# swishersnaaake/sexy-raytracer

Measured on AMD Instinct MI355X. Metric: Msamples/s (WxHxspp/s), 720p masterchief @5k spp, higher is better.
Workload: dtype f32; 1 GPU; masterchief_720p_5000spp; scene=masterchief, width=1280, height=720, spp=5000, max_bounce=4, seed=1, spp_chunks=625, tree=reference, traversal=faithful (bvh.h order), parallelism=tiles8x8 interleaved over 1 rank(s), 1 gather (none)

## Files before the change

sexy-raytracer_amd/csrc/srt_wavefront.hip:

```cpp
#include "srt_path.h"
#include "srt_launch.h"
#include "srt_wf_links.h"
#include "srt_wf_rings.h"

#define WF_BLOCK 1024
#define WF_SET_OF(mask) std::integral_constant<uint32_t, (mask)>()
#define WF_CTX_BYTES 128
#define WF_CTL_LIVE 28
#define WF_CTL_ABORT 29
#define WF_CTL_WORDS 64
#define WF_PEND_MISS 0
#define WF_PEND_TERMINAL 2

namespace {
enum { W_NODE = 0, W_PRIM = 1, W_SWAP = 2, W_SERVE = 3 };

__device__ __forceinline__ void bufStore4(Rsrc r, int off, float4 v) {
  u32x4 u;
  u.x = __float_as_uint(v.x); u.y = __float_as_uint(v.y); u.z = __float_as_uint(v.z); u.w = __float_as_uint(v.w);
  __builtin_amdgcn_raw_buffer_store_b128(u, r, off, 0, 0);
}
__device__ __forceinline__ void bufStore1(Rsrc r, int off, uint32_t v) { __builtin_amdgcn_raw_buffer_store_b32(v, r, off, 0, 0); }
typedef float f32x4 __attribute__((ext_vector_type(4)));
typedef __attribute__((address_space(3))) const f32x4 LdsVec4;
__device__ __forceinline__ uint32_t bufLoad1(Rsrc r, int off) { return __builtin_amdgcn_raw_buffer_load_b32(r, off, 0, 0); }
}

#define WF_PROF_KINDS 12
template <bool SINGLE, bool PROFILE, bool HYBRID, bool COUNT, bool MOMENTS = false>
__global__ __launch_bounds__(WF_BLOCK, 4) void srt_render_wf_kernel(const RenderArgs a) {
  static_assert(!(MOMENTS && (COUNT || PROFILE)), "the moments instances neither count nor profile");

  constexpr int32_t DONE = HYBRID ? -(1 << 29) : SRT_WF_DONE;
  constexpr int32_t DONE_PAIR = HYBRID ? (int32_t)0x80000000 : SRT_WF_DONE;
  typedef typename std::conditional<HYBRID, int32_t, uint16_t>::type PrimSlot;
  extern __shared__ int32_t lds[];
  const DevScene& sc = a.scene;
  char* const ldsTree = reinterpret_cast<char*>(lds);
  const int resident = HYBRID ? sc.wfResident : sc.numNodes;
  const int treeBytes = resident * 32;
  int32_t* const ctl = reinterpret_cast<int32_t*>(ldsTree + treeBytes);
  const int RCAP = a.wfRingCap, POOL = a.wfPoolSize;
  uint16_t* const ringSlots = reinterpret_cast<uint16_t*>(ctl + WF_CTL_WORDS);
  float* const hitT = reinterpret_cast<float*>(ringSlots + WF_RINGS * RCAP);
  PrimSlot* const hitPrim = reinterpret_cast<PrimSlot*>(hitT + POOL);
  const int lane = threadIdx.x & 63;
  const unsigned long long laneBelow = (1ull << lane) - 1ull;
  const uint64_t seedMixed = mix64(a.seed);
  const V3 background = ld3(a.background);
  const Rsrc rsNodes = makeRsrc(HYBRID ? sc.nodesWf : sc.nodes, sc.numNodes * 32);
  const Rsrc rsTris = makeRsrc(sc.triTest, HYBRID ? sc.numTris * 48 : 0);
  const Rsrc rsFast = makeRsrc(sc.triFast, HYBRID ? 0 : sc.numTris * 64);
  const Rsrc rsSpheres = makeRsrc(sc.spheres, sc.numSpheres * 48);
  const Rsrc rsTexels = makeRsrc(sc.texels, sc.texelBytes);
  const Rsrc rsClass = makeRsrc(sc.primClass, sc.numPrimClass);
  const Rsrc rsSecond = makeRsrc(sc.primSecond, HYBRID ? sc.numPrimClass * 4 : 0);
  const Rsrc rsPool = makeRsrc(a.wfPool + (size_t)blockIdx.x * POOL * WF_CTX_BYTES, POOL * WF_CTX_BYTES);
  const int hiLevels = a.maxBounce > 4 ? a.maxBounce - 4 : 0;
  const Rsrc rsAttHi = makeRsrc(a.wfAttHi + (size_t)blockIdx.x * 3 * hiLevels * POOL, 3 * hiLevels * POOL * 4);
  const bool singleRoot = SINGLE || sc.numWorld == 1;
  auto worldRef = [&](int k) {
    if (HYBRID) return sc.worldWf[k];
    return srtWfRootWord(sc.world[k]);
  };
  const SrtWfRingGeom ringGeom = {a.wfRingCap, a.wfRingShift, a.wfRingMul3};

  {
    float4* dst = reinterpret_cast<float4*>(ldsTree);
    for (int i = threadIdx.x; i < resident * 2; i += WF_BLOCK) {
      float4 v = bufLoad4(rsNodes, 16 * i);
      if (!HYBRID) {
        const int32_t thread = sc.nodeThread[i >> 1];
        v.w = __int_as_float((i & 1) ? srtWfMissWord(thread) : srtWfHitWord(__float_as_int(v.w), thread));
      }
      dst[i] = v;
    }
    for (int i = threadIdx.x; i < WF_CTL_WORDS; i += WF_BLOCK) ctl[i] = 0;
    for (int i = threadIdx.x; i < WF_RINGS * RCAP; i += WF_BLOCK) ringSlots[i] = 0;
    __syncthreads();
    for (int id = threadIdx.x; id < POOL; id += WF_BLOCK) ringSlots[WF_RING_NEWITEM * RCAP + id] = (uint16_t)(id + 1);
    if (threadIdx.x == 0) {
      ctl[WF_CTL_TAIL(WF_RING_NEWITEM)] = POOL;
      ctl[WF_CTL_LIVE] = POOL;
    }
    if (threadIdx.x < 16) ctl[threadIdx.x] = (int)(blockIdx.x % (unsigned)a.numQueues);
    __syncthreads();
  }
  int32_t* const waveQueue = ctl + (threadIdx.x >> 6);
  const int qHome = (int)(blockIdx.x % (unsigned)a.numQueues);
  const int unitItems = a.unitTiles * a.sppChunks * SRT_TILE_PIXELS;
  auto queueEnd = [&](int q) { return (q < a.numUnits ? (a.numUnits - q + a.numQueues - 1) / a.numQueues : 0) * unitItems; };

  auto raiseAbort = [&]() {
    if (__hip_atomic_exchange(&ctl[WF_CTL_ABORT], 1, __ATOMIC_RELAXED, WF_WG) == 0 && a.wfError) atomicAdd(a.wfError, 1);
  };
  auto enqueue = [&](auto set, int ring, int id) {
    if constexpr (HYBRID)
      srtWfEnqueueGeneric(ctl, ringSlots, ringGeom, lane, laneBelow, ring, id, raiseAbort);
    else
      srtWfEnqueue<decltype(set)::value>(ctl, ringSlots, ringGeom, lane, ring, id, raiseAbort);
  };

  int path = -1;
  int cur = DONE, hitRef = DONE, w = 0;
  int32_t link = DONE_PAIR;
  Ray ray;
  ray.o = ray.d = mk(0.0f, 0.0f, 0.0f);
  ray.time = 0.0f;
  float closest = SRT_INF, rayA = 0.0f, slabTol = SRT_INF;
  V3 rcpD = mk(0.0f, 0.0f, 0.0f), negOR = mk(0.0f, 0.0f, 0.0f);
  auto atNode = [&]() { return cur >= 0; };
  auto atPrim = [&]() { return (uint32_t)cur > (uint32_t)DONE; };
  unsigned long long cnt[8] = {0, 0, 0, 0, 0, 0, 0, 0};
  uint32_t walk0[4] = {0, 0, 0, 0};
  int aovPixel = -1;
  auto popNext = [&]() {
    int next;
    if (HYBRID) {
      const int follows = link & 3;
      next = link >> 2;
      if (follows == 1) next = cur - 2;
      if (follows == 2) next = (int)__builtin_amdgcn_raw_buffer_load_b32(rsSecond, (~cur) << 2, 0, 0);
      link &= ~3;
    } else {
      next = srtWfLeafHasSecond(cur) ? srtWfLeafRest(cur) : link;
    }
    if (!SINGLE && !singleRoot && next == DONE && ++w < sc.numWorld) {
      next = worldRef(w);
      link = DONE_PAIR;
    }
    cur = next;
  };
  auto startTraversal = [&]() {
    if constexpr (COUNT) {
      cnt[1]++;
      for (int k = 0; k < 4; ++k) walk0[k] = (uint32_t)cnt[2 + k];
    }
    rayA = lenSq(ray.d);
    const bool certified = (sc.fastDivScene != 0) & fastDivOperandOk(ray.o.x, ray.d.x) & fastDivOperandOk(ray.o.y, ray.d.y) &
                           fastDivOperandOk(ray.o.z, ray.d.z);
    rcpD = mk(refinedRcp(ray.d.x), refinedRcp(ray.d.y), refinedRcp(ray.d.z));
    slabSetup(ray.o, rcpD, certified, negOR, slabTol);
    closest = SRT_INF;
    hitRef = DONE;
    link = DONE_PAIR;
    w = 0;
    cur = worldRef(0);
  };
  auto cameraRayInto = [&](int at, uint32_t pxy, int s, float m1 = 0.0f, float m2 = 0.0f) {
    const int px = (int)(pxy & 0xffffu), py = (int)(pxy >> 16);
    Pcg rng;
    rng.key(seedMixed, (uint32_t)(py * a.imageWidth + px), (uint32_t)s);
    const float u = ((float)px + rng.uniform()) / (float)(a.imageWidth - 1);
    const float v = ((float)(a.imageHeight - py) + rng.uniform()) / (float)(a.imageHeight - 1);
    Ray r;
    const DevCamera cam = cameraFromKernarg();
    cameraRay(cam, u, v, rng, r);
    if constexpr (COUNT) cnt[0]++;
    bufStore4(rsPool, at, make_float4(r.o.x, r.o.y, r.o.z, r.time));
    bufStore4(rsPool, at + 16, make_float4(r.d.x, r.d.y, r.d.z, MOMENTS ? m1 : 0.0f));
    u32x4 Cn;
    Cn.x = (uint32_t)rng.state;
    Cn.y = (uint32_t)(rng.state >> 32);
    Cn.z = MOMENTS ? __float_as_uint(m2) : 0u;
    Cn.w = 0;
    __builtin_amdgcn_raw_buffer_store_b128(Cn, rsPool, at + 32, 0, 0);
  };

  int idleTrips = 0;
  uint32_t tick = 0;
  unsigned long long pCyc[WF_PROF_KINDS], pRuns[WF_PROF_KINDS], pLanes[WF_PROF_KINDS], pSched = 0;
  unsigned long long pSaw[8] = {0, 0, 0, 0, 0, 0, 0, 0};
  for (int k = 0; k < WF_PROF_KINDS; ++k) pCyc[k] = pRuns[k] = pLanes[k] = 0;
  const unsigned long long pStart = PROFILE ? clock64() : 0;
  unsigned long long pT = pStart;
  auto prof = [&](int kind, int lanes) {
    if (PROFILE) {
      const unsigned long long now = clock64();
      pCyc[kind] += now - pT;
      pRuns[kind]++;
      pLanes[kind] += lanes;
      pT = now;
    }
  };
  auto primStep = [&]() -> int {
    int nNodes;
      for (int round = 0; round < SRT_PRIM_ROUNDS; ++round) {
        if (round > 0 && __popcll(__ballot(atPrim())) < a.primAgainMin) break;
        if (PROFILE) {
          pRuns[1]++;
          pLanes[1] += __popcll(__ballot(atPrim()));
        }
        if (atPrim()) {
          const int ref = HYBRID ? cur : srtWfLeafFirst(cur);
          const int pr = ~ref;
          float t;
          bool ok;
          if (pr & 1) {
            if constexpr (COUNT) cnt[5]++;
            const int off = (pr >> 1) * 48;
            const float4 s0 = bufLoad4(rsSpheres, off), s1 = bufLoad4(rsSpheres, off + 16);
            V3 center = mk(s0.x, s0.y, s0.z);
            if (__float_as_int(s1.w) & (1 << 30)) {
              const float4 s2 = bufLoad4(rsSpheres, off + 32);
              center = center + ((ray.time - s2.x) / (s2.y - s2.x)) * (mk(s1.x, s1.y, s1.z) - center);
            }
            ok = sphereHitV(center, s0.w, ray, rayA, a.tMin, closest, t);
          } else {
            if constexpr (COUNT) cnt[4]++;
            if constexpr (HYBRID) {
              const int off = (pr >> 1) * 48;
              ok = triHitV<false>(bufLoad4(rsTris, off), bufLoad4(rsTris, off + 16), bufLoad4(rsTris, off + 32), ray, a.tMin, closest, t);
            } else {
              bool unsure;
              const int off = (pr >> 1) * 64;
              ok = srtTriHitCert(bufLoad4(rsFast, off), bufLoad4(rsFast, off + 16), bufLoad4(rsFast, off + 32), bufLoad4(rsFast, off + 48),
                                 triRay(ray), a.tMin, sc.triWMax, t, unsure);
              const unsigned long long mu = __ballot(unsure);
              if (PROFILE) {
                pRuns[11] += __popcll(mu);
                pCyc[11] += mu != 0 ? 1 : 0;
              }
              if (mu != 0) {
                if (unsure) {
                  const Rsrc rsExact = makeRsrc(sc.triTest, sc.numTris * 48);
                  const int at = (pr >> 1) * 48;
                  ok = triHitV<false>(bufLoad4(rsExact, at), bufLoad4(rsExact, at + 16), bufLoad4(rsExact, at + 32), ray, a.tMin, closest, t);
                }
              }
            }
          }
          if (ok) {
            closest = t;
            hitRef = ref;
          }
          popNext();
        }
      }
      nNodes = __popcll(__ballot(atNode()));
      if (PROFILE) {
        const unsigned long long now = clock64();
        pCyc[1] += now - pT;
        pT = now;
      }
      return nNodes;
  };
  auto nodeBurst = [&](int nNodes) -> int {
      const int keep = (nNodes * a.keepEighths) >> 3;
      int budget = a.nodeBurst, left;
      auto visit = [&](const float4 n0, const float4 n1) {
        bool undecided;
        bool hitBox = boxHitApprox<true>(n0, n1, rcpD, negOR, slabTol, a.tMin, closest, undecided);
        if (PROFILE) {
          const unsigned long long mu = __ballot(undecided);
          pLanes[8] += __popcll(mu);
          pLanes[7] += mu != 0 ? 1 : 0;
        }
        if (undecided) hitBox = boxHit(n0, n1, ray, a.tMin, closest);
        if constexpr (COUNT) {
          cnt[2]++;
          if (hitBox) cnt[3]++;
        }
        link = __float_as_int(n1.w);
        cur = hitBox ? __float_as_int(n0.w) : (HYBRID ? link >> 2 : link);
        if (!SINGLE && !singleRoot && cur == DONE && ++w < sc.numWorld) {
          cur = worldRef(w);
          link = DONE_PAIR;
        }
      };
      auto nodeVisit = [&](bool mine) {
        const bool here = HYBRID ? mine && (uint32_t)cur < (uint32_t)resident : cur >= 0;
        if (PROFILE) {
          pRuns[0]++;
          pLanes[0] += __popcll(__ballot(here));
        }
        if (here) {
          if constexpr (HYBRID) {
            const char* rec = ldsTree + (cur << 5);
            visit(*reinterpret_cast<const float4*>(rec), *reinterpret_cast<const float4*>(rec + 16));
          } else {
            const LdsVec4* rec = (const LdsVec4*)(uintptr_t)(uint32_t)cur;
            const f32x4 n0 = rec[0], n1 = rec[1];
            visit(make_float4(n0.x, n0.y, n0.z, n0.w), make_float4(n1.x, n1.y, n1.z, n1.w));
          }
        }
      };
      do {
        if (HYBRID) {
          const bool far = cur >= resident;
          float4 g0, g1;
          if (far) {
            g0 = bufLoad4(rsNodes, cur << 5);
            g1 = bufLoad4(rsNodes, (cur << 5) + 16);
          }
          if (a.wfFarRounds > 1) nodeVisit(!far);
          if (a.wfFarRounds > 2) nodeVisit(!far);
          if (a.wfFarRounds > 3) nodeVisit(!far);
          const bool near = !far && (uint32_t)cur < (uint32_t)resident;
          if (near) {
            const char* rec = ldsTree + (cur << 5);
            g0 = *reinterpret_cast<const float4*>(rec);
            g1 = *reinterpret_cast<const float4*>(rec + 16);
          }
          const unsigned long long f0 = PROFILE ? clock64() : 0;
          if (far || near) visit(g0, g1);
          if (PROFILE) {
            pRuns[10]++;
            pLanes[10] += __popcll(__ballot(far));
            pLanes[11] += __popcll(__ballot(near));
            pCyc[10] += clock64() - f0;
          }
        } else {
#pragma unroll
          for (int u = 0; u < SRT_NODE_UNROLL; ++u) nodeVisit(true);
        }
        budget -= HYBRID ? a.wfFarRounds : SRT_NODE_UNROLL;
        left = __popcll(__ballot(atNode()));
      } while (budget > 0 && left >= keep);
      if (PROFILE) {
        const unsigned long long now = clock64();
        pCyc[0] += now - pT;
        pT = now;
      }
      return left;
  };
  auto swapStep = [&]() {
      const bool fin = cur == DONE && path >= 0;
      const bool hit = fin && hitRef != DONE;
      const bool need = path < 0 || fin;
      const unsigned long long mNeed = __ballot(need);
      int id = -1;
      int cls = 0;
      if (hit) cls = (int)__builtin_amdgcn_raw_buffer_load_b8(rsClass, ~hitRef, 0, 0);
      const unsigned long long q0 = PROFILE ? clock64() : 0;
      if (mNeed != 0) {
        if constexpr (HYBRID)
          srtWfClaimGeneric(ctl, ringSlots, ringGeom, lane, laneBelow, WF_RING_READY, mNeed, __popcll(mNeed), 1, id, raiseAbort);
        else
          srtWfClaim(ctl, ringSlots, ringGeom, lane, WF_RING_READY, need, mNeed, __popcll(mNeed), 1, id, raiseAbort);
      }
      const unsigned long long q1 = PROFILE ? clock64() : 0;
      float4 A = make_float4(0.0f, 0.0f, 0.0f, 0.0f), B = A;
      if (id >= 0) {
        A = bufLoad4(rsPool, id << 7);
        B = bufLoad4(rsPool, (id << 7) + 16);
      }
      if (hit) {
        __hip_atomic_store(&hitT[path], closest, __ATOMIC_RELAXED, WF_WG);
        __hip_atomic_store(&hitPrim[path], (PrimSlot)hitRef, __ATOMIC_RELAXED, WF_WG);
      }
      asm volatile("" ::: "memory");
      enqueue(WF_SET_OF(WF_SET(WF_RING_RESTART) | WF_SET(WF_RING_HIT) | WF_SET(WF_RING_HIT + 1) | WF_SET(WF_RING_HIT + 2)),
              !fin ? -1 : (hit ? WF_RING_HIT + cls : WF_RING_RESTART), path);
      if constexpr (COUNT) {
        if (fin && aovPixel >= 0) {
          SrtAovRecord r;
          r.o[0] = ray.o.x; r.o[1] = ray.o.y; r.o[2] = ray.o.z;
          r.d[0] = ray.d.x; r.d[1] = ray.d.y; r.d[2] = ray.d.z;
          r.time = ray.time;
          r.valid = 1;
          r.prim = SRT_NO_HIT;
          r.t = 0.0f;
          if (hitRef != DONE) {
            const int pr = ~hitRef;
            r.prim = (pr & 1) ? sc.sphPrimId[pr >> 1] : sc.triPrimId[pr >> 1];
            r.t = closest;
          }
          r.nodeVisits = (int32_t)((uint32_t)cnt[2] - walk0[0]);
          r.boxPasses = (int32_t)((uint32_t)cnt[3] - walk0[1]);
          r.triTests = (int32_t)((uint32_t)cnt[4] - walk0[2]);
          r.sphereTests = (int32_t)((uint32_t)cnt[5] - walk0[3]);
          r.pad[0] = r.pad[1] = 0;
          a.aov[aovPixel] = r;
        }
      }
      if (fin) {
        path = -1;
        hitRef = DONE;
      }
      const unsigned long long q2 = PROFILE ? clock64() : 0;
      if (id >= 0) {
        ray.o = mk(A.x, A.y, A.z);
        ray.d = mk(B.x, B.y, B.z);
        ray.time = A.w;
        path = id;
        startTraversal();
        if constexpr (COUNT) {
          aovPixel = -1;
          if (a.aov) {
            const uint32_t cw = bufLoad1(rsPool, (id << 7) + 44);
            const u32x4 E = __builtin_amdgcn_raw_buffer_load_b128(rsPool, (id << 7) + 64, 0, 0);
            const int px = (int)(E.w & 0xffffu), py = (int)(E.w >> 16);
            if ((int)(cw & 0xffu) == a.aovDepth && (int)E.y == a.sampleFirst) aovPixel = py * a.imageWidth + px;
          }
        }
      }
      if (PROFILE) {
        const unsigned long long q3 = clock64();
        pSaw[5] += q1 - q0;
        pSaw[6] += q2 - q1;
        pSaw[7] += q3 - q2;
      }
      prof(2, __popcll(__ballot(fin)) + __popcll(__ballot(id >= 0)));
  };
  auto serveStep = [&](int bestRing, int serveAtLeast) -> int {
      int id;
      const unsigned long long h0 = PROFILE ? clock64() : 0;
      int k;
      if constexpr (HYBRID)
        k = srtWfClaimGeneric(ctl, ringSlots, ringGeom, lane, laneBelow, bestRing, ~0ull, 64, serveAtLeast, id, raiseAbort);
      else
        k = srtWfClaimAll(ctl, ringSlots, ringGeom, lane, bestRing, 64, serveAtLeast, id, raiseAbort);
      if (k == 0) {
        prof(8, 0);
        return 0;
      }
      const int at = id << 7;
      if (bestRing >= WF_RING_HIT && bestRing < WF_RING_HIT + WF_CLASSES) {
        bool toReady = false, toRestart = false;
        if (id >= 0) {
          const float4 A = bufLoad4(rsPool, at), B = bufLoad4(rsPool, at + 16);
          const u32x4 C = __builtin_amdgcn_raw_buffer_load_b128(rsPool, at + 32, 0, 0);
          const float tHit = __hip_atomic_load(&hitT[id], __ATOMIC_RELAXED, WF_WG);
          const int pr = HYBRID ? ~(int)__hip_atomic_load(&hitPrim[id], __ATOMIC_RELAXED, WF_WG)
                                : ~(int)(int16_t)__hip_atomic_load(&hitPrim[id], __ATOMIC_RELAXED, WF_WG);
          Ray rIn;
          rIn.o = mk(A.x, A.y, A.z);
          rIn.d = mk(B.x, B.y, B.z);
          rIn.time = A.w;
          Pcg rng;
          rng.state = (uint64_t)C.x | ((uint64_t)C.y << 32);
          int depth = (int)(C.w & 0xffu);
          Record rec;
          const unsigned long long h1 = PROFILE ? clock64() : 0;
          if (pr & 1)
            sphereRecord(sc, pr >> 1, rIn, tHit, rec, false);
          else
            triRecord(sc, pr >> 1, rIn, tHit, rec, false);
          V3 att, emitted;
          Ray next;
          uint32_t fetches = 0;
          if constexpr (COUNT) cnt[6] += rec.isTri ? 1 : 0;
          const unsigned long long h2 = PROFILE ? clock64() : 0;
          const bool scattered = shade<COUNT, true>(sc, rsTexels, rIn, rec, rng, att, next, emitted, fetches, nullptr);
          if constexpr (COUNT) cnt[7] += fetches;
          if (PROFILE && bestRing == WF_RING_HIT + 1) {
            const unsigned long long h3 = clock64();
            pSaw[1] += h1 - h0;
            pSaw[2] += h2 - h1;
            pSaw[3] += h3 - h2;
            pSaw[4] += 1;
          }
          V3 terminal = emitted;
          bool done = true;
          if (scattered) {
            if (depth < 4) {
              bufStore1(rsPool, at + 80 + 12 * depth, __float_as_uint(att.x));
              bufStore1(rsPool, at + 84 + 12 * depth, __float_as_uint(att.y));
              bufStore1(rsPool, at + 88 + 12 * depth, __float_as_uint(att.z));
            } else {
              const int slot = (3 * (depth - 4) * POOL + id) * 4;
              bufStore1(rsAttHi, slot, __float_as_uint(att.x));
              bufStore1(rsAttHi, slot + POOL * 4, __float_as_uint(att.y));
              bufStore1(rsAttHi, slot + POOL * 8, __float_as_uint(att.z));
            }
            depth++;
            done = depth >= a.maxBounce;
            terminal = mk(0.0f, 0.0f, 0.0f);
          }
          u32x4 Cn;
          Cn.x = (uint32_t)rng.state;
          Cn.y = (uint32_t)(rng.state >> 32);
          Cn.z = MOMENTS ? C.z : 0u;
          if (done) {
            bufStore4(rsPool, at + 16, make_float4(terminal.x, terminal.y, terminal.z, MOMENTS ? B.w : 0.0f));
            Cn.w = (uint32_t)depth | (WF_PEND_TERMINAL << 8);
            toRestart = true;
          } else {
            bufStore4(rsPool, at, make_float4(next.o.x, next.o.y, next.o.z, next.time));
            bufStore4(rsPool, at + 16, make_float4(next.d.x, next.d.y, next.d.z, MOMENTS ? B.w : 0.0f));
            Cn.w = (uint32_t)depth;
            toReady = true;
          }
          __builtin_amdgcn_raw_buffer_store_b128(Cn, rsPool, at + 32, 0, 0);
        }
        __builtin_amdgcn_fence(__ATOMIC_RELEASE, "workgroup");
        enqueue(WF_SET_OF(WF_SET(WF_RING_READY) | WF_SET(WF_RING_RESTART)), toReady ? WF_RING_READY : (toRestart ? WF_RING_RESTART : -1), id);
        prof(3 + bestRing - WF_RING_HIT, k);
      } else if (bestRing == WF_RING_RESTART) {
        bool toReady = false, toNewItem = false;
        if (id >= 0) {
          const float4 B = bufLoad4(rsPool, at + 16);
          const u32x4 C = __builtin_amdgcn_raw_buffer_load_b128(rsPool, at + 32, 0, 0);
          float4 D = bufLoad4(rsPool, at + 48);
          const u32x4 E = __builtin_amdgcn_raw_buffer_load_b128(rsPool, at + 64, 0, 0);
          const float4 F = bufLoad4(rsPool, at + 80), G = bufLoad4(rsPool, at + 96), H = bufLoad4(rsPool, at + 112);
          const int outIndex = (int)E.x, sEnd = (int)E.z;
          int s = (int)E.y;
          const int depth = (int)(C.w & 0xffu), pend = (int)((C.w >> 8) & 0xffu);
          V3 L = background;
          if (pend == WF_PEND_TERMINAL) L = mk(B.x, B.y, B.z);
          const float lv[12] = {F.x, F.y, F.z, F.w, G.x, G.y, G.z, G.w, H.x, H.y, H.z, H.w};
          for (int j = depth - 1; j >= 4; --j) {
            const int slot = (3 * (j - 4) * POOL + id) * 4;
            const float ax = __uint_as_float(bufLoad1(rsAttHi, slot)), ay = __uint_as_float(bufLoad1(rsAttHi, slot + POOL * 4)),
                        az = __uint_as_float(bufLoad1(rsAttHi, slot + POOL * 8));
            L = mk(0.0f + L.x * ax, 0.0f + L.y * ay, 0.0f + L.z * az);
          }
#pragma unroll
          for (int j = 3; j >= 0; --j)
            if (j < depth) L = mk(0.0f + L.x * lv[3 * j], 0.0f + L.y * lv[3 * j + 1], 0.0f + L.z * lv[3 * j + 2]);
          D.x += L.x;
          D.y += L.y;
          D.z += L.z;
          float m1 = 0.0f, m2 = 0.0f;
          if constexpr (MOMENTS) {
            const float l = sampleLum(L);
            m1 = B.w + l;
            m2 = __uint_as_float(C.z) + l * l;
          }
          s++;
          if (s < sEnd) {
            bufStore4(rsPool, at + 48, D);
            bufStore1(rsPool, at + 68, (uint32_t)s);
            if constexpr (MOMENTS)
              cameraRayInto(at, E.w, s, m1, m2);
            else
              cameraRayInto(at, E.w, s);
            toReady = true;
          } else {
            if (outIndex >= 0) {
              if (a.fix)
                commitFixed(a.fix + outIndex, mk(D.x, D.y, D.z), a.fixLimit);
              else
                a.out[outIndex] = D;
              if constexpr (MOMENTS) {
                if (a.mfix)
                  commitFixed(a.mfix + outIndex, mk(m1, m2, 0.0f), a.fixLimit);
                else
                  a.mout[outIndex] = make_float4(m1, m2, 0.0f, D.w);
              }
            }
            toNewItem = true;
          }
        }
        __builtin_amdgcn_fence(__ATOMIC_RELEASE, "workgroup");
        enqueue(WF_SET_OF(WF_SET(WF_RING_READY) | WF_SET(WF_RING_NEWITEM)), toReady ? WF_RING_READY : (toNewItem ? WF_RING_NEWITEM : -1), id);
        prof(6, k);
      } else {
        const bool need = id >= 0;
        const unsigned long long mF2 = __ballot(need);
        const int q = __builtin_amdgcn_readfirstlane(*waveQueue);
        bool gotItem = false, alive = true;
        int idx = 0;
        if (q >= 0) {
          int base = 0;
          if (lane == 0) base = atomicAdd(a.queue + 16 * q, __popcll(mF2));
          base = __builtin_amdgcn_readfirstlane(base);
          idx = HYBRID ? base + __popcll(mF2 & laneBelow) : (int)srtWfReservePlace((uint32_t)base, mF2, lane);
          const int qEnd = queueEnd(q);
          gotItem = need && idx < qEnd;
          if (base + __popcll(mF2) > qEnd) {
            int nq = -1;
            if (lane == 0) {
              int bestLeft = 0;
              bool bestOwn = false;
              for (int kq = 0; kq < a.numQueues; ++kq) {
                const int left = queueEnd(kq) - __hip_atomic_load(a.queue + 16 * kq, __ATOMIC_RELAXED, __HIP_MEMORY_SCOPE_AGENT);
                const bool own = ((kq ^ qHome) & 7) == 0;
                if (left > 0 && ((own && !bestOwn) || (own == bestOwn && left > bestLeft))) {
                  bestLeft = left;
                  bestOwn = own;
                  nq = kq;
                }
              }
              *waveQueue = nq;
            }
            nq = __builtin_amdgcn_readfirstlane(nq);
            if (nq < 0) alive = false;
          }
        } else {
          alive = false;
        }
        bool toReady = false, again = false, retired = false;
        if (need) {
          if (!gotItem) {
            retired = !alive;
            again = alive;
          } else {
            const int group = idx >> 6, ln = idx & 63;
            int u = (int)((float)group * a.rcpUnitGroups);
            int inUnit = group - u * a.unitGroups;
            if (inUnit < 0) {
              u--;
              inUnit += a.unitGroups;
            } else if (inUnit >= a.unitGroups) {
              u++;
              inUnit -= a.unitGroups;
            }
            int tileInUnit = (int)((float)inUnit * a.rcpChunks);
            int chunk = inUnit - tileInUnit * a.sppChunks;
            if (chunk < 0) {
              tileInUnit--;
              chunk += a.sppChunks;
            } else if (chunk >= a.sppChunks) {
              tileInUnit++;
              chunk -= a.sppChunks;
            }
            const int localTile = (q + u * a.numQueues) * a.unitTiles + tileInUnit;
            const int tile = a.tileFirst + localTile * a.tileStride;
            const uint32_t txy = a.tileXY[tile < a.numTiles ? tile : 0];
            const int px = (int)(txy & 0xffffu) * SRT_TILE_W + (ln & (SRT_TILE_W - 1));
            const int py = (int)(txy >> 16) * SRT_TILE_H + (ln >> 3);
            const uint32_t pxy = (uint32_t)px | ((uint32_t)py << 16);
            const int s0 = a.sampleFirst + chunk * a.sppBase + min(chunk, a.sppRem);
            const int s1 = s0 + a.sppBase + (chunk < a.sppRem ? 1 : 0);
            const bool valid = localTile < a.numLocalTiles && tile < a.numTiles && px < a.imageWidth && py < a.imageHeight && a.maxBounce > 0;
            const int outIndex = localTile < a.numLocalTiles ? chunk * a.chunkStride + localTile * SRT_TILE_PIXELS + ln : -1;
            const float4 D = make_float4(0.0f, 0.0f, 0.0f, (float)(s1 - s0));
            if (valid) {
              bufStore4(rsPool, at + 48, D);
              u32x4 En;
              En.x = (uint32_t)outIndex;
              En.y = (uint32_t)s0;
              En.z = (uint32_t)s1;
              En.w = pxy;
              __builtin_amdgcn_raw_buffer_store_b128(En, rsPool, at + 64, 0, 0);
              cameraRayInto(at, pxy, s0);
              toReady = true;
            } else {
              if (outIndex >= 0 && !a.fix) a.out[outIndex] = D;
              if constexpr (MOMENTS) {
                if (outIndex >= 0 && !a.mfix) a.mout[outIndex] = D;
              }
              again = true;
            }
          }
        }
        __builtin_amdgcn_fence(__ATOMIC_RELEASE, "workgroup");
        enqueue(WF_SET_OF(WF_SET(WF_RING_READY) | WF_SET(WF_RING_NEWITEM)), toReady ? WF_RING_READY : (again ? WF_RING_NEWITEM : -1), id);
        const unsigned long long mR = __ballot(retired);
        if (mR != 0 && lane == __ffsll((long long)mR) - 1) __hip_atomic_fetch_sub(&ctl[WF_CTL_LIVE], __popcll(mR), __ATOMIC_RELAXED, WF_WG);
        prof(9, k);
      }
      return k;
  };
  auto flushProfile = [&]() {
  if (PROFILE && a.stats && lane == 0) {
      for (int k = 0; k < WF_PROF_KINDS; ++k) {
        atomicAdd(&a.stats[32 + k], pCyc[k]);
        atomicAdd(&a.stats[32 + WF_PROF_KINDS + k], pRuns[k]);
        atomicAdd(&a.stats[32 + 2 * WF_PROF_KINDS + k], pLanes[k]);
      }
      atomicAdd(&a.stats[32 + 3 * WF_PROF_KINDS], pSched);
      atomicAdd(&a.stats[32 + 3 * WF_PROF_KINDS + 1], (unsigned long long)(clock64() - pStart));
      for (int k = 0; k < 8; ++k) atomicAdd(&a.stats[32 + 3 * WF_PROF_KINDS + 2 + k], pSaw[k]);
    }
  };
  bool traverseFirst = false;
  for (;;) {
    int nN, nP, free, nNknown = -1;
    for (;;) {
      nN = nNknown >= 0 ? nNknown : __popcll(__ballot(atNode()));
      nP = __popcll(__ballot(atPrim()));
      free = 64 - nN - nP;
      if (nN + nP == 0) break;
      if (!traverseFirst && (free >= a.wfSwapMin || (++tick & 3u) == 0)) break;
      traverseFirst = false;
      if (PROFILE) {
        const unsigned long long now = clock64();
        pSched += now - pT;
        pT = now;
      }
      if (nP >= a.primMin || nN == 0) {
        const int nNodes = primStep();
        nNknown = nNodes >= a.fuseMin ? nodeBurst(nNodes) : nNodes;
      } else {
        nNknown = nodeBurst(nN);
      }
    }
    const int nF = __popcll(__ballot(cur == DONE && path >= 0));
    int pick, serveAtLeast = 64, bestRing = WF_RING_RESTART;
    {
      unsigned long long* cw = reinterpret_cast<unsigned long long*>(ctl + 16);
      const unsigned long long w0 = __hip_atomic_load(cw + 0, __ATOMIC_RELAXED, WF_WG), w1 = __hip_atomic_load(cw + 1, __ATOMIC_RELAXED, WF_WG),
                               w2 = __hip_atomic_load(cw + 2, __ATOMIC_RELAXED, WF_WG), w3 = __hip_atomic_load(cw + 3, __ATOMIC_RELAXED, WF_WG),
                               w4 = __hip_atomic_load(cw + 4, __ATOMIC_RELAXED, WF_WG), w5 = __hip_atomic_load(cw + 5, __ATOMIC_RELAXED, WF_WG),
                               w6 = __hip_atomic_load(cw + 6, __ATOMIC_RELAXED, WF_WG);
      if ((int)(w6 >> 32) != 0) break;
      auto fill = [](unsigned long long th) { return (int)((uint32_t)th - (uint32_t)(th >> 32)); };
      const int readyAvail = __builtin_amdgcn_readfirstlane(fill(w0));
      const int av[5] = {fill(w1), fill(w2), fill(w3), fill(w4), fill(w5)};
      int bestAvail = av[0];
#pragma unroll
      for (int r = 1; r < 5; ++r)
        if (av[r] > bestAvail) {
          bestAvail = av[r];
          bestRing = WF_RING_RESTART + r;
        }
      bestRing = __builtin_amdgcn_readfirstlane(bestRing);
      bestAvail = __builtin_amdgcn_readfirstlane(bestAvail);
      const int swapGain = nF + (readyAvail < free ? readyAvail : free);
      if (bestAvail >= 64)
        pick = W_SERVE;
      else if (swapGain >= a.wfSwapMin)
        pick = W_SWAP;
      else if (nP >= a.primMin || (nN == 0 && nP > 0))
        pick = W_PRIM;
      else if (nN > 0)
        pick = W_NODE;
      else if (swapGain > 0)
        pick = W_SWAP;
      else if (bestAvail > 0) {
        pick = W_SERVE;
        serveAtLeast = 1;
      } else {
        if (__builtin_amdgcn_readfirstlane((int)w6) <= 0) break;
        if (++idleTrips > WF_SPIN_LIMIT) {
          raiseAbort();
          break;
        }
        __builtin_amdgcn_s_sleep(8);
        prof(7, 0);
        continue;
      }
      idleTrips = 0;
      if (PROFILE) {
        pSaw[0]++;
        (void)readyAvail;
      }
    }
    if (PROFILE) {
      const unsigned long long now = clock64();
      pSched += now - pT;
      pT = now;
    }

    if (pick == W_PRIM || pick == W_NODE) {
      traverseFirst = true;
    } else if (pick == W_SWAP) {
      swapStep();
    } else if (pick == W_SERVE) {
      serveStep(bestRing, serveAtLeast);
    }
  }
  flushProfile();
  if constexpr (COUNT) {
    if (a.stats) {
      for (int k = 0; k < 8; ++k) {
        unsigned long long x = cnt[k];
        for (int off = 32; off > 0; off >>= 1) x += __shfl_down(x, off);
        if (lane == 0) atomicAdd(&a.stats[k], x);
      }
    }
  }
}

extern "C" {
RenderKernel srt_render_wf_kernel_for(const RenderPlan* p) {
  static_assert(WF_BLOCK == SRT_BLOCK_TREE, "srt_render.cpp launches the path-pool kernel with SRT_BLOCK_TREE threads");
  if (p->moments) {
    if (p->form == 4) return p->single ? srt_render_wf_kernel<true, false, true, false, true> : srt_render_wf_kernel<false, false, true, false, true>;
    return p->single ? srt_render_wf_kernel<true, false, false, false, true> : srt_render_wf_kernel<false, false, false, false, true>;
  }
  if (p->form == 4)
    return p->count     ? (p->single ? srt_render_wf_kernel<true, false, true, true> : srt_render_wf_kernel<false, false, true, true>)
           : p->profile ? srt_render_wf_kernel<false, true, true, false>
                        : (p->single ? srt_render_wf_kernel<true, false, true, false> : srt_render_wf_kernel<false, false, true, false>);
  return p->count     ? (p->single ? srt_render_wf_kernel<true, false, false, true> : srt_render_wf_kernel<false, false, false, true>)
         : p->profile ? srt_render_wf_kernel<false, true, false, false>
                      : (p->single ? srt_render_wf_kernel<true, false, false, false> : srt_render_wf_kernel<false, false, false, false>);
}
}
```

Before: 5897 Msamples/s.

## Overlap serve-step pool loads with a window of LDS node visits

In the non-hybrid path, serveStep now issues its global pool buffer loads (hit ring, restart ring) or the queue atomicAdd up front. When enough lanes are still at a node, it then runs one unrolled round of four LDS node visits before consuming those results, so traversal work hides the memory latency. This raises register pressure because many float4 values stay live across the node visits, and it changes the interleaving of traversal with serving.

```diff
diff --git a/sexy-raytracer_amd/csrc/srt_wavefront.hip b/sexy-raytracer_amd/csrc/srt_wavefront.hip
--- a/sexy-raytracer_amd/csrc/srt_wavefront.hip
+++ b/sexy-raytracer_amd/csrc/srt_wavefront.hip
@@ -11,6 +11,9 @@
 #define WF_CTL_WORDS 64
 #define WF_PEND_MISS 0
 #define WF_PEND_TERMINAL 2
+#ifndef SRT_WF_WINDOW_MIN
+#define SRT_WF_WINDOW_MIN 8
+#endif
 
 namespace {
 enum { W_NODE = 0, W_PRIM = 1, W_SWAP = 2, W_SERVE = 3 };
@@ -22,6 +25,7 @@
 }
 __device__ __forceinline__ void bufStore1(Rsrc r, int off, uint32_t v) { __builtin_amdgcn_raw_buffer_store_b32(v, r, off, 0, 0); }
 typedef float f32x4 __attribute__((ext_vector_type(4)));
+typedef unsigned int u32x2 __attribute__((ext_vector_type(2)));
 typedef __attribute__((address_space(3))) const f32x4 LdsVec4;
 __device__ __forceinline__ uint32_t bufLoad1(Rsrc r, int off) { return __builtin_amdgcn_raw_buffer_load_b32(r, off, 0, 0); }
 }
@@ -245,7 +249,7 @@
       }
       return nNodes;
   };
-  auto nodeBurst = [&](int nNodes) -> int {
+  auto nodeBurst = [&](int nNodes, auto window) -> int {
       const int keep = (nNodes * a.keepEighths) >> 3;
       int budget = a.nodeBurst, left;
       auto visit = [&](const float4 n0, const float4 n1) {
@@ -285,6 +289,14 @@
           }
         }
       };
+      if constexpr (decltype(window)::value) {
+        static_assert(SRT_NODE_UNROLL == 4, "the window is one burst round");
+        nodeVisit(true);
+        nodeVisit(true);
+        nodeVisit(true);
+        nodeVisit(true);
+        return 0;
+      }
       do {
         if (HYBRID) {
           const bool far = cur >= resident;
@@ -403,7 +415,7 @@
       }
       prof(2, __popcll(__ballot(fin)) + __popcll(__ballot(id >= 0)));
   };
-  auto serveStep = [&](int bestRing, int serveAtLeast) -> int {
+  auto serveStep = [&](int bestRing, int serveAtLeast, int nN) -> int {
       int id;
       const unsigned long long h0 = PROFILE ? clock64() : 0;
       int k;
@@ -416,14 +428,68 @@
         return 0;
       }
       const int at = id << 7;
-      if (bestRing >= WF_RING_HIT && bestRing < WF_RING_HIT + WF_CLASSES) {
+      const bool hitRing = bestRing >= WF_RING_HIT && bestRing < WF_RING_HIT + WF_CLASSES;
+      float4 fA, fB, fD, fF, fG, fH;
+      u32x4 fC, fE;
+      float fT;
+      int fPr, fBase, fQ = -1;
+      unsigned long long fNeed = 0;
+      if constexpr (!HYBRID) {
+        if (hitRing) {
+          if (id >= 0) {
+            fT = __hip_atomic_load(&hitT[id], __ATOMIC_RELAXED, WF_WG);
+            fPr = ~(int)(int16_t)__hip_atomic_load(&hitPrim[id], __ATOMIC_RELAXED, WF_WG);
+            fA = bufLoad4(rsPool, at);
+            fB = bufLoad4(rsPool, at + 16);
+            fC = __builtin_amdgcn_raw_buffer_load_b128(rsPool, at + 32, 0, 0);
+          }
+        } else if (bestRing == WF_RING_RESTART) {
+          if (id >= 0) {
+            fB = bufLoad4(rsPool, at + 16);
+            if constexpr (MOMENTS) {
+              const u32x2 c = __builtin_amdgcn_raw_buffer_load_b64(rsPool, at + 40, 0, 0);
+              fC.z = c.x;
+              fC.w = c.y;
+            } else {
+              fC.w = bufLoad1(rsPool, at + 44);
+            }
+            fD = bufLoad4(rsPool, at + 48);
+            fE = __builtin_amdgcn_raw_buffer_load_b128(rsPool, at + 64, 0, 0);
+            fF = bufLoad4(rsPool, at + 80);
+            fG = bufLoad4(rsPool, at + 96);
+            fH = bufLoad4(rsPool, at + 112);
+          }
+        } else {
+          fNeed = __ballot(id >= 0);
+          fQ = __builtin_amdgcn_readfirstlane(*waveQueue);
+          int zero = 0;
+          asm volatile("" : "+v"(zero));
+          if (fQ >= 0 && lane == 0) fBase = atomicAdd(a.queue + 16 * fQ + zero, __popcll(fNeed));
+        }
+        if (nN >= SRT_WF_WINDOW_MIN) {
+          nodeBurst(nN, std::true_type());
+        }
+      }
+      if (hitRing) {
         bool toReady = false, toRestart = false;
         if (id >= 0) {
-          const float4 A = bufLoad4(rsPool, at), B = bufLoad4(rsPool, at + 16);
-          const u32x4 C = __builtin_amdgcn_raw_buffer_load_b128(rsPool, at + 32, 0, 0);
-          const float tHit = __hip_atomic_load(&hitT[id], __ATOMIC_RELAXED, WF_WG);
-          const int pr = HYBRID ? ~(int)__hip_atomic_load(&hitPrim[id], __ATOMIC_RELAXED, WF_WG)
-                                : ~(int)(int16_t)__hip_atomic_load(&hitPrim[id], __ATOMIC_RELAXED, WF_WG);
+          float4 A, B;
+          u32x4 C;
+          float tHit;
+          int pr;
+          if constexpr (!HYBRID) {
+            A = fA;
+            B = fB;
+            C = fC;
+            tHit = fT;
+            pr = fPr;
+          } else {
+            A = bufLoad4(rsPool, at);
+            B = bufLoad4(rsPool, at + 16);
+            C = __builtin_amdgcn_raw_buffer_load_b128(rsPool, at + 32, 0, 0);
+            tHit = __hip_atomic_load(&hitT[id], __ATOMIC_RELAXED, WF_WG);
+            pr = ~(int)__hip_atomic_load(&hitPrim[id], __ATOMIC_RELAXED, WF_WG);
+          }
           Ray rIn;
           rIn.o = mk(A.x, A.y, A.z);
           rIn.d = mk(B.x, B.y, B.z);
@@ -471,7 +537,7 @@
           u32x4 Cn;
           Cn.x = (uint32_t)rng.state;
           Cn.y = (uint32_t)(rng.state >> 32);
-          Cn.z = MOMENTS ? C.z : 0u;
+          Cn.z = MOMENTS || !HYBRID ? C.z : 0u;
           if (done) {
             bufStore4(rsPool, at + 16, make_float4(terminal.x, terminal.y, terminal.z, MOMENTS ? B.w : 0.0f));
             Cn.w = (uint32_t)depth | (WF_PEND_TERMINAL << 8);
@@ -490,11 +556,19 @@
       } else if (bestRing == WF_RING_RESTART) {
         bool toReady = false, toNewItem = false;
         if (id >= 0) {
-          const float4 B = bufLoad4(rsPool, at + 16);
-          const u32x4 C = __builtin_amdgcn_raw_buffer_load_b128(rsPool, at + 32, 0, 0);
-          float4 D = bufLoad4(rsPool, at + 48);
-          const u32x4 E = __builtin_amdgcn_raw_buffer_load_b128(rsPool, at + 64, 0, 0);
-          const float4 F = bufLoad4(rsPool, at + 80), G = bufLoad4(rsPool, at + 96), H = bufLoad4(rsPool, at + 112);
+          float4 B, D, F, G, H;
+          u32x4 C, E;
+          if constexpr (!HYBRID) {
+            B = fB; C = fC; D = fD; E = fE; F = fF; G = fG; H = fH;
+          } else {
+            B = bufLoad4(rsPool, at + 16);
+            C = __builtin_amdgcn_raw_buffer_load_b128(rsPool, at + 32, 0, 0);
+            D = bufLoad4(rsPool, at + 48);
+            E = __builtin_amdgcn_raw_buffer_load_b128(rsPool, at + 64, 0, 0);
+            F = bufLoad4(rsPool, at + 80);
+            G = bufLoad4(rsPool, at + 96);
+            H = bufLoad4(rsPool, at + 112);
+          }
           const int outIndex = (int)E.x, sEnd = (int)E.z;
           int s = (int)E.y;
           const int depth = (int)(C.w & 0xffu), pend = (int)((C.w >> 8) & 0xffu);
@@ -549,13 +623,17 @@
         prof(6, k);
       } else {
         const bool need = id >= 0;
-        const unsigned long long mF2 = __ballot(need);
-        const int q = __builtin_amdgcn_readfirstlane(*waveQueue);
+        const unsigned long long mF2 = HYBRID ? __ballot(need) : fNeed;
+        const int q = HYBRID ? __builtin_amdgcn_readfirstlane(*waveQueue) : fQ;
         bool gotItem = false, alive = true;
         int idx = 0;
         if (q >= 0) {
           int base = 0;
-          if (lane == 0) base = atomicAdd(a.queue + 16 * q, __popcll(mF2));
+          if constexpr (HYBRID) {
+            if (lane == 0) base = atomicAdd(a.queue + 16 * q, __popcll(mF2));
+          } else {
+            base = fBase;
+          }
           base = __builtin_amdgcn_readfirstlane(base);
           idx = HYBRID ? base + __popcll(mF2 & laneBelow) : (int)srtWfReservePlace((uint32_t)base, mF2, lane);
           const int qEnd = queueEnd(q);
@@ -674,9 +752,9 @@
       }
       if (nP >= a.primMin || nN == 0) {
         const int nNodes = primStep();
-        nNknown = nNodes >= a.fuseMin ? nodeBurst(nNodes) : nNodes;
+        nNknown = nNodes >= a.fuseMin ? nodeBurst(nNodes, std::false_type()) : nNodes;
       } else {
-        nNknown = nodeBurst(nN);
+        nNknown = nodeBurst(nN, std::false_type());
       }
     }
     const int nF = __popcll(__ballot(cur == DONE && path >= 0));
@@ -741,7 +819,7 @@
     } else if (pick == W_SWAP) {
       swapStep();
     } else if (pick == W_SERVE) {
-      serveStep(bestRing, serveAtLeast);
+      serveStep(bestRing, serveAtLeast, nN);
     }
   }
   flushProfile();
```

Result: no change. 5948 Msamples/s (median of 6 runs) (+0.9%).
